# jackra1n/raytracer-rust

Measured on AMD Instinct MI355X. Metric: Msamples/s (pixels x spp / s) at 800x600x256spp; 1/2/4/8-GPU scaling, higher is better.
Workload: dtype f32; 1 GPU; cornell-box-800x600x256-d30; scene=data/scenes/tungsten/cornell-box/scene.json, width=800, height=600, spp=256, max_bounces=30, parallelism=row strips of 4 dealt round-robin over 1 GPU(s), frames_in_flight=1

## Files before the change

raytracer-rust_amd/csrc/device/rt_api.cpp:

```cpp
#include <hip/hip_runtime_api.h>

#include <algorithm>
#include <cmath>
#include <cstdio>
#include <cstdlib>
#include <cstring>
#include <map>
#include <mutex>
#include <new>
#include <stdexcept>
#include <string>
#include <thread>
#include <vector>

#include "../../../include/mi355rt.h"
#include "rt_device.h"
#include "rt_host.h"
#include "rt_query.h"

using namespace mi355rt;

namespace {

void row_tables(const std::vector<uint32_t>& rows, const std::vector<float>& cost, uint32_t groups, std::vector<uint32_t>& out) {
// ... 38 lines not shown
    uint32_t inline_steps = 0;
    uint32_t trav_min = 24;
    bool have_scene = false;
    mi355rt_settings settings{};
    DevCamera cam{};
    float miss[3] = {0.5f, 0.5f, 0.5f};
    uint32_t n_prims = 0, n_mats = 0; size_t n_nodes = 0;
    DevBuf<DevPrim> prims; DevBuf<DevMat> mats; DevBuf<DevNode> nodes; DevBuf<DevTri> tris;
    DevBuf<uint32_t> rows; DevBuf<float> radiance; DevBuf<uint32_t> counters; DevBuf<unsigned long long> stats;
    DevBuf<float> fold_stack;
    DevBuf<float> sky; uint32_t sky_w = 0, sky_h = 0;
    DevBuf<DevTexture> textures; DevBuf<uint32_t> texels;
    DevBuf<unsigned long long> wave_times; uint32_t wave_times_n = 0;
    std::vector<uint32_t> rows_host;
    std::vector<uint32_t> tables_host;
    bool rows_valid = false;
    std::vector<float> row_cost;
    int knob_row_order = -1;
    uint32_t order_groups = 0;
    hipEvent_t ev[3] = {nullptr, nullptr, nullptr};
    hipEvent_t done = nullptr; hipStream_t last_stream = nullptr; bool have_last = false;
    bool want_wave_times = false;
    DevBuf<unsigned long long> errword; unsigned long long* h_err = nullptr; unsigned long long err_reported = 0;
    uint32_t spin_limit_idle = SPIN_LIMIT_IDLE, spin_limit_entry = SPIN_LIMIT_ENTRY;
    uint32_t launched_variants = 0;
    int forced_variant = -1;
    int knob_inline_steps = -1;
    bool timing = false;
    std::vector<hipEvent_t> pool; size_t pool_used = 0;
    uint32_t timed_launches = 0;
// ... 24 lines not shown
    ctx->launched_variants = 0;
    for (const auto& w : waits) if ((now >> 32) & w.bit) which += std::string(which.empty() ? "" : "; ") + w.what;
    return fail(MI355RT_ERR_HIP, "kernel watchdog: " + std::to_string(n) + " wave(s) gave up a bounded wait " + (this_render ? "in this render" : "in an earlier render on this context") +
                                 " -- that image is incomplete [kernel(s) launched on this context since the last report: " + (kernels.empty() ? "?" : kernels) + "; wait: " + (which.empty() ? "?" : which) +
                                 "; limits: " + std::to_string(ctx->spin_limit_idle) + " idle polls, " + std::to_string(ctx->spin_limit_entry) + " polls of a ring entry]");
}

namespace {

uint32_t built_variants() {
    uint32_t mask = 0u;
    for (uint32_t v = 0; v < KERNEL_VARIANTS; ++v) if (render_ctr_variant_built(v)) mask |= 1u << v;
    return mask;
}

int build_device_scene(mi355rt_context* ctx, const mi355rt_scene* sc) {
    PreparedScene s;
    int rc = prepare_scene(sc, s); if (rc) return rc;
    const bool has_sky = sc->sky_rgb != nullptr;
    if ((rc = ctx->prims.ensure(s.prims.size()))) return rc;
    if ((rc = ctx->mats.ensure(sc->n_materials))) return rc;
    if ((rc = ctx->nodes.ensure(s.nodes.size()))) return rc;
    if ((rc = ctx->tris.ensure(s.tris.size()))) return rc;
    static_assert(sizeof(DevMat) == sizeof(mi355rt_material), "material layout is shared with the ABI");
    if (!s.prims.empty()) HIP_TRY(hipMemcpy(ctx->prims.p, s.prims.data(), s.prims.size() * sizeof(DevPrim), hipMemcpyHostToDevice));
    if (sc->n_materials) HIP_TRY(hipMemcpy(ctx->mats.p, sc->materials, sc->n_materials * sizeof(DevMat), hipMemcpyHostToDevice));
    if (!s.nodes.empty()) HIP_TRY(hipMemcpy(ctx->nodes.p, s.nodes.data(), s.nodes.size() * sizeof(DevNode), hipMemcpyHostToDevice));
    if (!s.tris.empty()) HIP_TRY(hipMemcpy(ctx->tris.p, s.tris.data(), s.tris.size() * sizeof(DevTri), hipMemcpyHostToDevice));
    ctx->n_prims = sc->n_primitives; ctx->n_mats = sc->n_materials; ctx->n_nodes = s.nodes.size();
    std::memcpy(ctx->miss, sc->miss_color, 12);
    ctx->sky_w = ctx->sky_h = 0;
// ... 8 lines not shown
        if ((rc = ctx->textures.ensure(sc->n_textures))) return rc;
        std::vector<DevTexture> table(sc->n_textures);
        size_t off = 0;
        for (uint32_t i = 0; i < sc->n_textures; ++i) {
            const mi355rt_texture& t = sc->textures[i];
            const size_t n = (size_t)t.width * t.height;
            HIP_TRY(hipMemcpy(ctx->texels.p + off, t.rgba8, n * 4, hipMemcpyHostToDevice));
            table[i] = DevTexture{ctx->texels.p + off, t.width, t.height};
            off += n;
        }
        HIP_TRY(hipMemcpy(ctx->textures.p, table.data(), table.size() * sizeof(DevTexture), hipMemcpyHostToDevice));
    }
    ctx->has_mesh = s.n_mesh_prims != 0;
    ctx->variant = choose_variant(s, ctx->forced_variant, built_variants());
    ctx->inline_steps = choose_inline_steps(s, ctx->knob_inline_steps);
    return MI355RT_OK;
}

std::mutex g_knob_mutex;
std::map<std::string, int> g_default_knobs;
int apply_knob(mi355rt_context* ctx, const std::string& name, int v) {
    if (name == "kernel") { if (v < -1 || v >= (int)KERNEL_VARIANTS) return fail(MI355RT_ERR_INVALID, "knob kernel"); ctx->forced_variant = v; }
    else if (name == "inline_steps") { if (v < -1 || v > 8) return fail(MI355RT_ERR_INVALID, "knob inline_steps"); ctx->knob_inline_steps = v; }
    else if (name == "grid_div") { if (v < 1 || v > 16) return fail(MI355RT_ERR_INVALID, "knob grid_div"); ctx->grid_div = (uint32_t)v; }
    else if (name == "guided_mult") { if (v < 1 || v > 64) return fail(MI355RT_ERR_INVALID, "knob guided_mult"); ctx->guided_mult = (uint32_t)v; }
    else if (name == "trav_min") { if (v < 1 || v > 64) return fail(MI355RT_ERR_INVALID, "knob trav_min"); ctx->trav_min = (uint32_t)v; }
    else if (name == "spin_idle") { if (v < 1) return fail(MI355RT_ERR_INVALID, "knob spin_idle"); ctx->spin_limit_idle = (uint32_t)v; }
    else if (name == "spin_entry") { if (v < 1) return fail(MI355RT_ERR_INVALID, "knob spin_entry"); ctx->spin_limit_entry = (uint32_t)v; }
    else if (name == "wave_times") ctx->want_wave_times = v != 0;
    else if (name == "row_order") { if (v < -1 || v > 1) return fail(MI355RT_ERR_INVALID, "knob row_order"); ctx->knob_row_order = v; }
    else return fail(MI355RT_ERR_INVALID, "unknown knob " + name);
    return MI355RT_OK;
}

}

extern "C" {

int mi355rt_debug_set_knob(mi355rt_context* ctx, const char* name, int value) {
    return guard([&]() -> int {
    if (ctx) return name ? apply_knob(ctx, name, value) : fail(MI355RT_ERR_INVALID, "knob name is null");
    std::lock_guard<std::mutex> g(g_knob_mutex);
    if (!name) { g_default_knobs.clear(); return MI355RT_OK; }
    mi355rt_context probe;
// ... 62 lines not shown
    delete ctx;
}

static int render_samples(mi355rt_context* ctx, const mi355rt_options* opt, uint32_t s0, uint32_t s1, void* d_accum,
                          void* d_out_packed, void* d_out_linear, void* hip_stream, mi355rt_stats* stats, unsigned long long* d_row_counters = nullptr);

int mi355rt_context_set_scene(mi355rt_context* ctx, const mi355rt_scene* scene, const mi355rt_camera* camera,
                              const mi355rt_settings* settings) {
    return guard([&]() -> int {
    if (!ctx) return fail(MI355RT_ERR_INVALID, "ctx is null");
    if (!camera) return fail(MI355RT_ERR_INVALID, "camera is null");
    int rc = check_settings(settings); if (rc) return rc;
    HIP_TRY(hipSetDevice(ctx->device));
    ctx->have_scene = false; ctx->rows_valid = false;
    ctx->query_rows_release();
    rc = build_device_scene(ctx, scene); if (rc) return rc;
    static_assert(sizeof(DevCamera) == sizeof(mi355rt_camera), "camera layout is shared with the ABI");
    std::memcpy(&ctx->cam, camera, sizeof(DevCamera));
    ctx->settings = *settings;
    ctx->have_scene = true;
    struct TimingOff { mi355rt_context* c; bool was; ~TimingOff() { c->timing = was; } } timing_off{ctx, ctx->timing};
    ctx->timing = false;
    struct ProbeScope {
        mi355rt_context* c; mi355rt_settings full; uint32_t variant; uint32_t* d_tmp = nullptr; unsigned long long* d_cnt = nullptr; bool committed = false;
        ProbeScope(mi355rt_context* ctx) : c(ctx), full(ctx->settings), variant(ctx->variant) {}
        ~ProbeScope() {
            c->settings = full; c->rows_valid = false;
            if (d_tmp) (void)hipFree(d_tmp);
            if (d_cnt) (void)hipFree(d_cnt);
            if (!committed) { c->variant = variant; c->have_scene = false; c->row_cost.clear(); }
        }
// ... 52 lines not shown
    if (ctx->have_last && ctx->last_stream != stream) HIP_TRY(hipStreamWaitEvent(stream, ctx->done, 0));
    const uint32_t rng_mode = opt ? opt->rng_mode : (uint32_t)MI355RT_RNG_CTR;
    uint32_t groups = WORK_SHARDS;
    {   const uint64_t spp_now = std::max<uint64_t>(1, (uint64_t)s1 - s0), pixels = (uint64_t)sel.rows.size() * st.width;
        const uint64_t ws = (opt && opt->workspace_bytes) ? opt->workspace_bytes : (32ull << 30);
        const uint64_t cap = std::max<uint64_t>(1, std::min<uint64_t>(ws / 12, (1ull << 31) - 16 * RUN_LIMIT) / spp_now);
        const uint64_t band_pixels = std::max<uint64_t>(1, std::min(cap, pixels));
        groups *= (uint32_t)std::min<uint64_t>(64, std::max<uint64_t>(1, (pixels + band_pixels - 1) / band_pixels)); }
    if (ctx->row_cost.empty() || rng_mode != MI355RT_RNG_CTR) groups = 0;
    const bool same_rows = ctx->rows_valid && sel.rows == ctx->rows_host && groups == ctx->order_groups;
    if (!same_rows) {
        if (ctx->have_last) HIP_TRY(hipEventSynchronize(ctx->done));
        ctx->rows_host.swap(sel.rows);
        static const std::vector<float> no_cost;
        row_tables(ctx->rows_host, groups ? ctx->row_cost : no_cost, groups, ctx->tables_host);
        ctx->order_groups = groups;
        ctx->rows_valid = false;
    }
    const bool fixed_aabb = opt && (opt->flags & MI355RT_FLAG_FIXED_AABB) != 0u;
    if (opt && (opt->flags & ~MI355RT_FLAG_FIXED_AABB) != 0u) return fail(MI355RT_ERR_INVALID, "options.flags has unknown bits");
    if (fixed_aabb && rng_mode != MI355RT_RNG_CTR) return fail(MI355RT_ERR_INVALID, "MI355RT_FLAG_FIXED_AABB needs MI355RT_RNG_CTR (the replay mode reproduces the reference as it is)");
    uint32_t variant = ctx->variant;
    if (fixed_aabb && ctx->has_mesh) variant = VARIANT_TABLE[variant].fixed_aabb;
    if ((ctx->n_prims == 0 || st.max_depth == 0) && VARIANT_TABLE[variant].family == FAMILY_LOCKSTEP && !(VARIANT_TABLE[variant].prims & (1u << MI355RT_PRIM_MESH)))
        variant = KERNEL_LOCKSTEP_MESH;
    const uint64_t seed = opt ? opt->seed : 0;
    const uint32_t n_rows = (uint32_t)ctx->rows_host.size();
    if (stats) { std::memset(stats, 0, sizeof *stats); stats->rows_rendered = n_rows; stats->kernel_vgprs = (uint32_t)ctx->vgprs[variant]; stats->kernel_sgprs = (uint32_t)ctx->sgprs; }
    if (n_rows == 0) return MI355RT_OK;

    if (!same_rows) {
        if ((rc = ctx->rows.ensure(3 * (size_t)n_rows))) return rc;
        HIP_TRY(hipMemcpyAsync(ctx->rows.p, ctx->tables_host.data(), 3 * (size_t)n_rows * sizeof(uint32_t), hipMemcpyHostToDevice, stream));
        ctx->rows_valid = true;
    }
    const uint32_t* d_rows_natural = ctx->rows.p;
    const uint32_t* d_rows_processing = ctx->rows.p + n_rows;
    const uint32_t* d_out_row = ctx->order_groups ? ctx->rows.p + 2 * (size_t)n_rows : nullptr;
    if ((rc = ctx->stats.ensure(STATS_WORDS))) return rc;
    HIP_TRY(hipMemsetAsync(ctx->stats.p, 0, STATS_WORDS * sizeof(unsigned long long), stream));

    double render_ms = 0, resolve_ms = 0, total_ms = 0;
    uint32_t n_bands = 0, grid_blocks = 0, block_threads = 0;

    if (rng_mode == MI355RT_RNG_REF) {
        if (d_accum || s0 != 0 || s1 != st.samples_per_pixel)
            return fail(MI355RT_ERR_INVALID, "progressive rendering needs MI355RT_RNG_CTR (the reference stream of a row is sequential over its pixels)");
        if ((rc = ctx->fold_stack.ensure((size_t)n_rows * std::max(st.max_depth, 1u) * 3))) return rc;
// ... 36 lines not shown

        RenderParams p{};
        p.prims = ctx->prims.p; p.mats = ctx->mats.p; p.nodes = ctx->nodes.p; p.tris = ctx->tris.p; p.rows = d_rows_processing;
        p.sky = ctx->sky_w ? ctx->sky.p : nullptr; p.sky_w = ctx->sky_w; p.sky_h = ctx->sky_h; p.textures = ctx->textures.p;
        p.radiance = ctx->radiance.p; p.stats = ctx->stats.p;
        p.n_prims = ctx->n_prims; p.n_mats = ctx->n_mats;
        std::memcpy(p.miss, ctx->miss, 12); p.cam = ctx->cam;
        p.width = st.width; p.height = st.height; p.spp = (uint32_t)spp; p.max_depth = st.max_depth;
        p.width_f = (float)st.width; p.height_f = (float)st.height;
        { volatile float one = 1.0f; p.inv_width_rn = one / p.width_f; p.inv_height_rn = one / p.height_f; }
        p.seed_lo = (uint32_t)seed; p.seed_hi = (uint32_t)(seed >> 32); p.sample0 = s0;
        magic_div((uint32_t)spp, p.spp_mul, p.spp_shift); magic_div(st.width, p.width_mul, p.width_shift);
        p.trav_min = ctx->trav_min; p.inline_steps = ctx->inline_steps;
        p.lds_nodes = (uint32_t)std::min<size_t>(ctx->n_nodes, LDS_NODE_CAP);
        p.err = ctx->errword.p; p.spin_limit_idle = ctx->spin_limit_idle; p.spin_limit_entry = ctx->spin_limit_entry;
        ResolveParams r{};
        r.radiance = ctx->radiance.p; r.out_packed = (uint32_t*)d_out_packed; r.out_linear = (float*)d_out_linear;
        r.spp = (uint32_t)spp; r.inv_spp = 1.0f / (float)s1;
        r.accum = (float*)d_accum; r.accum_load = s0 != 0 ? 1u : 0u;
        r.out_row = d_out_row; r.width = st.width; r.width_mul = p.width_mul; r.width_shift = p.width_shift;
        const uint32_t resident = std::max(1u, (uint32_t)(ctx->cu_count * ctx->blocks_per_cu[variant]) / ctx->grid_div);
        block_threads = VARIANT_TABLE[variant].block_threads;
        std::vector<float> band_ms;
        for (uint32_t b = 0; b < n_bands; ++b) {
            const uint64_t p0 = (uint64_t)b * band_pixels_max;
            const uint64_t np = std::min<uint64_t>(band_pixels_max, total_pixels - p0);
            p.band_pixel0 = (uint32_t)p0; p.band_samples = (uint32_t)(np * spp);
            p.batch_counter = ctx->counters.p + (size_t)b * ctr_words;
            if (d_row_counters) p.stats = d_row_counters + STATS_WORDS * (size_t)b;
            const bool wf = VARIANT_TABLE[variant].family == FAMILY_WAVEFRONT;
// ... 178 lines not shown
    if (!out_variant || !out_inline_steps || !n_prims || !n_nodes || !n_tris) return fail(MI355RT_ERR_INVALID, "debug_prepare_scene: null");
    if (forced_variant < -1 || forced_variant >= (int)KERNEL_VARIANTS) return fail(MI355RT_ERR_INVALID, "knob kernel");
    PreparedScene s;
    const int rc = prepare_scene(scene, s); if (rc) return rc;
    if ((prims && *n_prims < s.prims.size()) || (nodes && *n_nodes < s.nodes.size()) || (tris && *n_tris < s.tris.size())) return fail(MI355RT_ERR_INVALID, "debug_prepare_scene: capacity");
    if (prims && !s.prims.empty()) std::memcpy(prims, s.prims.data(), s.prims.size() * sizeof(DevPrim));
    if (nodes && !s.nodes.empty()) std::memcpy(nodes, s.nodes.data(), s.nodes.size() * sizeof(DevNode));
    if (tris && !s.tris.empty()) std::memcpy(tris, s.tris.data(), s.tris.size() * sizeof(DevTri));
    *n_prims = (uint32_t)s.prims.size(); *n_nodes = (uint32_t)s.nodes.size(); *n_tris = (uint32_t)s.tris.size();
    *out_variant = choose_variant(s, forced_variant, built_variants());
    *out_inline_steps = choose_inline_steps(s, -1);
    return MI355RT_OK;
    });
}

int mi355rt_debug_read_counters(mi355rt_context* ctx, unsigned long long* out40) {
    return guard([&]() -> int {
    if (!ctx || !out40 || !ctx->stats.p) return fail(MI355RT_ERR_INVALID, "no counters");
    HIP_TRY(hipSetDevice(ctx->device));
    HIP_TRY(hipMemcpy(out40, ctx->stats.p, STATS_WORDS * sizeof(unsigned long long), hipMemcpyDeviceToHost));
    return MI355RT_OK;
    });
}

int mi355rt_debug_read_row_tables(mi355rt_context* ctx, uint32_t* tables, uint32_t capacity_entries, uint32_t* n_rows, float* cost, uint32_t cost_capacity, uint32_t* n_cost) {
    return guard([&]() -> int {
    if (!ctx || !n_rows) return fail(MI355RT_ERR_INVALID, "null");
    const size_t n = ctx->rows_host.size();
    *n_rows = (uint32_t)n;
    if (tables) { if (capacity_entries < 3 * n || ctx->tables_host.size() != 3 * n) return fail(MI355RT_ERR_INVALID, "row tables: capacity"); std::memcpy(tables, ctx->tables_host.data(), 3 * n * sizeof(uint32_t)); }
// ... 248 lines not shown
```

raytracer-rust_amd/csrc/device/rt_device.h:

```cpp
#pragma once
#include <stdint.h>
#include "../../../include/mi355rt.h"

namespace mi355rt {

struct DevPrim {
    uint32_t kind, material, node_begin, run_end;
    float d[52];
    float mat0[4];
};
static_assert(sizeof(DevPrim) == 240, "DevPrim must stay 16-byte granular");
static_assert(offsetof(DevPrim, d) % 16 == 0, "DevPrim::d is read sixteen words at a time as a 16-byte aligned vector (rt_intersect.h load_rec16)");

struct DevMat {
    uint32_t kind; float albedo[3];
    float aux[3];  float p0;
    float p1;      float eta[3];
    float k[3];    uint32_t texture;
};
static_assert(sizeof(DevMat) == 64, "DevMat");

struct DevTexture { const uint32_t* rgba8; uint32_t width, height; };

struct DevNode { float bmin[3]; uint32_t a; float bmax[3]; uint32_t b; };
// ... 31 lines not shown
    DevCamera cam;
    uint32_t width, height, spp, max_depth;
    float width_f, height_f, inv_width_rn, inv_height_rn;
    uint32_t band_pixel0;
    uint32_t band_samples;
    uint32_t guided_div;
    uint32_t shard_samples;
    uint32_t seed_lo, seed_hi;
    uint32_t sample0;
    uint32_t spp_mul, spp_shift, width_mul, width_shift;
    uint32_t trav_min;
    uint32_t inline_steps;
    uint32_t lds_nodes;
    uint32_t spin_limit_idle;
    uint32_t spin_limit_entry;
};
enum : uint32_t { WAIT_WF_IDLE = 1u, WAIT_WF_RING = 2u, WAIT_WF_FOLLOWED = 4u };
constexpr uint32_t SPIN_LIMIT_IDLE = 1u << 22;
constexpr uint32_t SPIN_LIMIT_ENTRY = 1u << 20;

enum : uint32_t {
    KERNEL_LOCKSTEP = 0, KERNEL_LOCKSTEP_MESH = 1, KERNEL_STATE_MACHINE = 2, KERNEL_LOCKSTEP_SIMPLE = 3, KERNEL_STATE_MACHINE_FIXAABB = 4,
    KERNEL_RETIRED_5 = 5, KERNEL_RETIRED_6 = 6, KERNEL_WAVEFRONT = 7, KERNEL_WAVEFRONT_FIXAABB = 8, KERNEL_LOCKSTEP_NOSPEC = 9,
    KERNEL_WAVEFRONT_NOMETAL = 10, KERNEL_WAVEFRONT_MESHFREE = 11, KERNEL_WAVEFRONT_NOMETAL_IDENT = 12, KERNEL_WAVEFRONT_NOMETAL_SHALLOW = 13,
    KERNEL_LOCKSTEP_SIMPLE_QC = 14, KERNEL_VARIANTS = 15
};
constexpr uint32_t PRIMS_ALL = 0xFFFFFFFFu;
constexpr uint32_t PRIMS_MESH_FREE = PRIMS_ALL & ~(1u << MI355RT_PRIM_MESH);
constexpr uint32_t PRIMS_QUAD_CUBE = (1u << MI355RT_PRIM_QUAD) | (1u << MI355RT_PRIM_CUBE);
constexpr uint32_t WF_SHALLOW_NODES = 4096;
constexpr uint32_t MATBIT(uint32_t kind) { return 1u << kind; }
// ... 105 lines not shown
```

raytracer-rust_amd/csrc/device/rt_intersect.h:

```cpp
#pragma once
#include "rt_math.h"

namespace mi355rt {

struct Hit { float t; f3 p; f3 n; uint32_t mat_ff; float4 q0; };
constexpr uint32_t CAND_NONE = 0xFFFFFFFFu;
struct Cand {
    float t;
    uint32_t idx;
    float aux;
    uint32_t aux2;
};
DI void cand_reset(Cand& c) { c.t = __builtin_inff(); c.idx = CAND_NONE; c.aux = 0.f; c.aux2 = 0u; }
struct CandP : Cand { f3 po; };
DI void cand_reset(CandP& c) { cand_reset(static_cast<Cand&>(c)); c.po = mk(0.f, 0.f, 0.f); }

DI void set_face(Hit& h, f3 rd, f3 outward, uint32_t material) {
    bool front = dot(rd, outward) < 0.0f;
    h.n = front ? outward : -outward;
    h.mat_ff = material | (front ? 0x80000000u : 0u);
}

struct Probe { float t, aux; f3 po; };
typedef float rec16_t __attribute__((ext_vector_type(16), aligned(16)));
// ... 278 lines not shown
            set_face(h, rd, divf(h.p - mk(pr->d[0], pr->d[1], pr->d[2]), pr->d[3]), pr->material);
        } else if (kind == MI355RT_PRIM_PLANE) {
            h.p = ro + rd * c.t;
            set_face(h, rd, mk(pr->d[3], pr->d[4], pr->d[5]), pr->material);
        } else if (HAS_MESH) {
            f3 outward; finish_mesh(pr, reinterpret_cast<const float4*>(tris), c, ro, rd, h.p, outward);
            set_face(h, rd, outward, pr->material);
        }
    }
}

#undef MI_KIND
DI uint32_t prim_material_kind(const RenderParams& P, uint32_t idx) { return __float_as_uint(P.prims[idx].mat0[0]); }

template <bool HAS_MESH, uint32_t KINDS = PRIMS_ALL, class C>
DI void walk_list(cprim_t prims, uint32_t n_prims, const DevNode* __restrict__ nodes, const DevTri* __restrict__ tris, f3 ro, f3 rd, C& c) {
#define MI_KIND(k) (((KINDS >> (k)) & 1u) != 0u)
    uint32_t i = 0;
    while (i < n_prims) {
#define MI_RUN(KIND, CALL) if (i < n_prims && prims[i].kind == (KIND)) { const uint32_t end = min(prims[i].run_end, n_prims); do { CALL; } while (++i < end); }
        if (MI_KIND(MI355RT_PRIM_QUAD)) { MI_RUN(MI355RT_PRIM_QUAD,   hit_quad<!HAS_MESH>(prims + i, i, ro, rd, EPS, c)) }
        if (MI_KIND(MI355RT_PRIM_CUBE)) { MI_RUN(MI355RT_PRIM_CUBE,   hit_cube<!HAS_MESH>(prims + i, i, ro, rd, EPS, c)) }
        if (MI_KIND(MI355RT_PRIM_SPHERE)) { MI_RUN(MI355RT_PRIM_SPHERE, hit_sphere(prims + i, i, ro, rd, EPS, c)) }
        if (MI_KIND(MI355RT_PRIM_PLANE)) { MI_RUN(MI355RT_PRIM_PLANE,  hit_plane(prims + i, i, ro, rd, EPS, c)) }
        if (HAS_MESH) { MI_RUN(MI355RT_PRIM_MESH, hit_mesh(prims + i, i, nodes, tris, ro, rd, EPS, c)) }
        else if (KINDS == PRIMS_ALL) { if (i < n_prims && prims[i].kind >= MI355RT_PRIM_MESH) ++i; }
        else if (i < n_prims && ((KINDS >> prims[i].kind) & 1u) == 0u) ++i;
#undef MI_RUN
#undef MI_KIND
    }
}
template <bool HAS_MESH, bool CARRY_PO = false, uint32_t KINDS = PRIMS_ALL>
DI bool hit_scene(cprim_t prims, uint32_t n_prims, const DevNode* __restrict__ nodes, const DevTri* __restrict__ tris,
                  f3 ro, f3 rd, Hit& best) {
    typename std::conditional<CARRY_PO && !HAS_MESH, CandP, Cand>::type c; cand_reset(c);
    walk_list<HAS_MESH, KINDS>(prims, n_prims, nodes, tris, ro, rd, c);
    if (c.idx == CAND_NONE) return false;
    finish_hit<HAS_MESH, !HAS_MESH, !HAS_MESH, KINDS>((const DevPrim*)prims, tris, c, ro, rd, best);
    return true;
}


}
```

raytracer-rust_amd/csrc/device/rt_kernels.hip:

```cpp
#include <hip/hip_runtime.h>
#include <stdint.h>
#include <type_traits>
#include "rt_device.h"
#include "../../../include/mi355rt.h"

#include "rt_math.h"
#include "rt_rng.h"
#include "rt_intersect.h"
#include "rt_materials.h"

namespace mi355rt {

DI uint32_t mbcnt64(uint64_t mask) { return __builtin_amdgcn_mbcnt_hi((uint32_t)(mask >> 32), __builtin_amdgcn_mbcnt_lo((uint32_t)mask, 0u)); }
DI uint32_t wave_sum(uint32_t v) {
#pragma unroll
    for (int off = 32; off > 0; off >>= 1) v += __shfl_xor(v, off, 64);
    return v;
}
template <bool FENCED = true>
DI void wave_lds_handoff() {
    if constexpr (FENCED) __builtin_amdgcn_fence(__ATOMIC_RELEASE, "wavefront", "local");
    __builtin_amdgcn_wave_barrier();
    if constexpr (FENCED) __builtin_amdgcn_fence(__ATOMIC_ACQUIRE, "wavefront", "local");
}
// ... 376 lines not shown
    stock.dir = s_stock_dir + (threadIdx.x & ~63u); stock.key = s_stock_key + (threadIdx.x & ~63u);
    }
    PathState ps; ps.ro = mk(0, 0, 0); ps.rd = mk(0, 0, 1); ps.thr = mk(1, 1, 1); ps.sidx = 0; ps.ray_index = 0; ps.px = ps.py = 0;
    ps.rng.clear();
    bool live = false;
    uint32_t n_paths = 0, n_rays = 0;
    Prof prof; prof.begin();
#ifdef MI355RT_STAMPS
    const unsigned long long t_wave0 = __builtin_amdgcn_s_memrealtime();
    unsigned long long t_dry = 0ull; uint32_t drain_iters = 0, live_at_dry = 0;
#endif
    for (;;) {
        Hit h; bool hit = false;
        __builtin_amdgcn_s_setprio(1);
        uint32_t n_cam = 0u;
        if constexpr (PREHIT) {
            n_cam = wc.template refill_size<MI355RT_PREHIT_LOW>(P, lane);
            if (n_cam != 0u) {
                wave_lds_handoff();
                stock.park_a[lane] = make_float4(ps.ro.x, ps.ro.y, ps.ro.z, ps.rd.x); stock.park_b[lane] = make_float2(ps.rd.y, ps.rd.z);
                if (lane < n_cam) stock.camera(P, wc.next + lane, (wc.ring_head + wc.ring_count + lane) & 63u, ps.ro, ps.rd);
            }
        }
        if (n_cam != 0u ? lane < n_cam : live) hit = hit_scene<HAS_MESH, true, KINDS>(prims, P.n_prims, P.nodes, P.tris, ps.ro, ps.rd, h);
        prof.mark(1);
        if constexpr (PREHIT) {
            if (n_cam != 0u) {
                const bool cam = lane < n_cam;
                if (cam) { ++n_paths; ++n_rays; }
                wave_lds_handoff();
                wc.ring_count += stock.append(P, lane, wc.next, wc.ring_head + wc.ring_count, cam, hit, h, ps.rd);
                wave_lds_handoff();
                wc.next += n_cam;
                const float4 a = stock.park_a[lane]; const float2 b = stock.park_b[lane];
                ps.ro = mk(a.x, a.y, a.z); ps.rd = mk(a.w, b.x, b.y);
                prof.mark(2);
                continue;
            }
        }
// ... 246 lines not shown
```

raytracer-rust_amd/csrc/device/rt_prepare.cpp:

```cpp
#include "rt_prepare.h"

#include <algorithm>
#include <cmath>
#include <cstring>
#include <initializer_list>
#include <limits>
#include <utility>

using namespace mi355rt;

namespace {
thread_local std::string g_err;
}

namespace mi355rt {

int fail(int code, const std::string& msg) { g_err = msg; return code; }
int fail_noexcept(int code, const char* msg) noexcept { try { g_err.assign(msg); } catch (...) { g_err.clear(); } return code; }
std::string& last_error() { return g_err; }

int select_rows(const mi355rt_settings& st, const mi355rt_options* o, RowSel& sel) {
    uint32_t rb = 0, re = st.height, strip = 1, parts = 1, part = 0;
    if (o) {
        if (o->abi_version != MI355RT_ABI_VERSION && o->abi_version != 4u) return fail(MI355RT_ERR_INVALID, "options.abi_version mismatch");
// ... 260 lines not shown
                     : (rough && other_scatter && covers(KERNEL_WAVEFRONT_MESHFREE)) ? KERNEL_WAVEFRONT_MESHFREE
                     : covers(KERNEL_LOCKSTEP_NOSPEC) ? KERNEL_LOCKSTEP_NOSPEC : KERNEL_LOCKSTEP;
    }
    if (forced_variant >= 0) {
        const uint32_t v = (uint32_t)forced_variant;
        const bool ok = render_ctr_variant_built(v) && VARIANT_TABLE[v].forceable && covers(v) && kinds_covered(v) &&
                        !(VARIANT_TABLE[v].identity_meshes && !(has_mesh && all_meshes_identity));
        if (ok) chosen = v;
    }
    return chosen;
}

uint32_t choose_inline_steps(const PreparedScene& s, int knob) { return knob >= 0 ? (uint32_t)knob : (s.n_mesh_prims >= 2 ? 1u : 0u); }

}
```

raytracer-rust_amd/csrc/device/rt_prepare.h:

```cpp
#pragma once

#include <cstdint>
#include <new>
#include <stdexcept>
#include <string>
#include <vector>

#include "../../../include/mi355rt.h"
#include "rt_device.h"

namespace mi355rt {

int fail(int code, const std::string& msg);
int fail_noexcept(int code, const char* msg) noexcept;
std::string& last_error();

template <class F> int guard(F&& f) noexcept {
    try { return f(); }
    catch (const std::bad_alloc&) { return fail_noexcept(MI355RT_ERR_OOM, "host allocation failed (std::bad_alloc)"); }
    catch (const std::length_error&) { return fail_noexcept(MI355RT_ERR_OOM, "host allocation failed (std::length_error)"); }
    catch (const std::exception& e) {
        try { return fail(MI355RT_ERR_HIP, std::string("unexpected C++ exception: ") + e.what()); } catch (...) { return fail_noexcept(MI355RT_ERR_HIP, "unexpected C++ exception"); }
    }
    catch (...) { return fail_noexcept(MI355RT_ERR_HIP, "unexpected C++ exception"); }
// ... 7 lines not shown
struct PreparedScene {
    std::vector<DevNode> nodes; std::vector<DevTri> tris;
    std::vector<uint32_t> mesh_roots;
    std::vector<DevPrim> prims;
    uint64_t n_texels = 0;
    uint32_t scene_mats = 0u;
    uint32_t scene_prim_kinds = 0u;
    uint32_t n_mesh_prims = 0;
    bool all_meshes_identity = true, all_meshes_shallow = true;
};

int prepare_scene(const mi355rt_scene* sc, PreparedScene& out);
uint32_t choose_variant(const PreparedScene& s, int forced_variant, uint32_t built_mask);
uint32_t choose_inline_steps(const PreparedScene& s, int knob);

}
```

raytracer-rust_amd/device.py:

```python
import collections
import ctypes as C
import os

import numpy as np

from . import abi, build

EXPORTS = ["mi355rt_render", "mi355rt_render_multi", "mi355rt_render_progressive", "mi355rt_context_create", "mi355rt_context_destroy", "mi355rt_context_set_scene",
           "mi355rt_rows_selected", "mi355rt_context_render", "mi355rt_context_render_progressive", "mi355rt_context_set_timing", "mi355rt_context_read_timing",
           "mi355rt_context_check", "mi355rt_context_set_share", "mi355rt_last_error", "mi355rt_abi_version",
           "mi355rt_multi_context_create", "mi355rt_multi_context_destroy", "mi355rt_multi_context_set_scene", "mi355rt_multi_context_render",
           "mi355rt_multi_context_check", "mi355rt_multi_context_render_progressive", "mi355rt_render_progressive_multi",
           "mi355rt_context_trace_rays", "mi355rt_context_first_hits", "mi355rt_trace_rays"]

_lib = None
_extra = {}


def load(so):
    so = os.path.abspath(so)
    if so not in _extra:
        _extra[so] = _bind(so)
    return _extra[so]

# ... 126 lines not shown
        L.mi355rt_context_trace_rays.restype = C.c_int
        L.mi355rt_context_trace_rays.argtypes = [C.c_void_p, C.c_void_p, C.c_uint32, C.c_void_p, C.c_void_p]
        L.mi355rt_context_first_hits.restype = C.c_int
        L.mi355rt_context_first_hits.argtypes = [C.c_void_p, C.POINTER(abi.Options), C.c_void_p, C.c_void_p]
        L.mi355rt_trace_rays.restype = C.c_int
        L.mi355rt_trace_rays.argtypes = [C.POINTER(abi.Scene), C.c_void_p, C.c_uint32, C.c_void_p]
        L.mi355rt_debug_multi_part_ms.restype = C.c_int
        L.mi355rt_debug_multi_part_ms.argtypes = [C.c_void_p, C.POINTER(C.c_double), C.c_uint32, C.POINTER(C.c_uint32)]
        L.mi355rt_debug_set_knob.restype = C.c_int
        L.mi355rt_debug_set_knob.argtypes = [C.c_void_p, C.c_char_p, C.c_int]
        L.mi355rt_debug_has_variant.restype = C.c_int
        L.mi355rt_debug_has_variant.argtypes = [C.c_uint32]
        L.mi355rt_debug_prepare_scene.restype = C.c_int
        L.mi355rt_debug_prepare_scene.argtypes = [C.POINTER(abi.Scene), C.c_int, C.POINTER(C.c_uint32), C.POINTER(C.c_uint32),
                                                  C.c_void_p, C.POINTER(C.c_uint32), C.c_void_p, C.POINTER(C.c_uint32), C.c_void_p, C.POINTER(C.c_uint32)]
        if L.mi355rt_abi_version() != abi.ABI_VERSION:
            raise RuntimeError("libmi355rt.so ABI version does not match abi.py")
    return L


class RenderError(RuntimeError):
    def __init__(self, what, rc, library=None):
        super().__init__(f"{what} failed ({rc}): {(library or lib()).mi355rt_last_error().decode()}")
        self.rc = rc


def _check(rc, what, library=None):
    if rc != 0:
        raise RenderError(what, rc, library)

# ... 12 lines not shown
NODE_DTYPE = np.dtype([("bmin", "<f4", 3), ("a", "<u4"), ("bmax", "<f4", 3), ("b", "<u4")])
TRI_DTYPE = np.dtype([("v0", "<f4", 3), ("e1", "<f4", 3), ("e2", "<f4", 3), ("n", "<f4", 3)])
Prepared = collections.namedtuple("Prepared", "variant inline_steps prims nodes tris")


def prepare_scene(scene, forced_variant=-1, library=None):
    L = library or lib()
    sc = getattr(scene, "c", scene)
    variant, inline_steps, n_prims, n_nodes, n_tris = (C.c_uint32() for _ in range(5))
    _check(L.mi355rt_debug_prepare_scene(C.byref(sc), int(forced_variant), C.byref(variant), C.byref(inline_steps), None, C.byref(n_prims),
                                         None, C.byref(n_nodes), None, C.byref(n_tris)), "mi355rt_debug_prepare_scene", L)
    prims, nodes, tris = np.zeros(n_prims.value, PRIM_DTYPE), np.zeros(n_nodes.value, NODE_DTYPE), np.zeros(n_tris.value, TRI_DTYPE)
    _check(L.mi355rt_debug_prepare_scene(C.byref(sc), int(forced_variant), C.byref(variant), C.byref(inline_steps), prims.ctypes.data, C.byref(n_prims),
                                         nodes.ctypes.data, C.byref(n_nodes), tris.ctypes.data, C.byref(n_tris)), "mi355rt_debug_prepare_scene", L)
    return Prepared(variant.value, inline_steps.value, prims, nodes, tris)


def render(scene, camera, settings, options=None, want_linear=True, want_stats=True, library=None):
    L = library or lib()
    sc = getattr(scene, "c", scene)
    rows = len(abi.rows_selected(settings.height, options))
    W = settings.width
    packed = np.zeros((rows, W), np.uint32)
    linear = np.zeros((rows, W, 3), np.float32) if want_linear else None
    stats = abi.Stats() if want_stats else None
    _check(L.mi355rt_render(C.byref(sc), C.byref(camera), C.byref(settings),
                            C.byref(options) if options is not None else None,
                            packed.ctypes.data, linear.ctypes.data if want_linear else None,
                            C.byref(stats) if want_stats else None), "mi355rt_render", L)
    return packed, linear, stats
# ... 261 lines not shown
```

Measured before the change: 10270 Msamples/s.

## Cull primitives for camera rays using per-pixel projected coverage masks

Adds a host-side pass that projects each quad and cube primitive's corners into screen space and builds a per-pixel 32-bit mask of primitives that could be hit by primary rays. The masks are gathered per processed row, uploaded alongside the row tables, and used in the lockstep kernel to skip intersection tests for primitives not covering the pixel range of a camera-ray refill. This cuts per-ray intersection work on the first bounce for small scenes like the Cornell box. It adds a host pass and an upload of width-by-rows words, plus a scalar mask load per refill, and relies on conservative inflation and dilation to stay correct.

```diff
diff --git a/raytracer-rust_amd/csrc/device/rt_api.cpp b/raytracer-rust_amd/csrc/device/rt_api.cpp
--- a/raytracer-rust_amd/csrc/device/rt_api.cpp
+++ b/raytracer-rust_amd/csrc/device/rt_api.cpp
@@ -76,6 +76,8 @@
     DevBuf<unsigned long long> wave_times; uint32_t wave_times_n = 0;
     std::vector<uint32_t> rows_host;
     std::vector<uint32_t> tables_host;
+    std::vector<uint32_t> cam_mask_abs, cam_mask_host; uint32_t cam_mask_w = 0, cam_mask_h = 0;
+    int knob_cam_cull = -1;
     bool rows_valid = false;
     std::vector<float> row_cost;
     int knob_row_order = -1;
@@ -130,7 +132,7 @@
     return mask;
 }
 
-int build_device_scene(mi355rt_context* ctx, const mi355rt_scene* sc) {
+int build_device_scene(mi355rt_context* ctx, const mi355rt_scene* sc, const mi355rt_camera* camera, const mi355rt_settings* st) {
     PreparedScene s;
     int rc = prepare_scene(sc, s); if (rc) return rc;
     const bool has_sky = sc->sky_rgb != nullptr;
@@ -169,6 +171,13 @@
     ctx->has_mesh = s.n_mesh_prims != 0;
     ctx->variant = choose_variant(s, ctx->forced_variant, built_variants());
     ctx->inline_steps = choose_inline_steps(s, ctx->knob_inline_steps);
+    ctx->cam_mask_abs.clear(); ctx->cam_mask_host.clear();
+    if (ctx->variant == KERNEL_LOCKSTEP_SIMPLE_QC && ctx->knob_cam_cull != 0) {
+        static_assert(sizeof(DevCamera) == sizeof(mi355rt_camera), "camera layout is shared with the ABI");
+        DevCamera cam; std::memcpy(&cam, camera, sizeof cam);
+        build_camera_masks(s, cam, st->width, st->height, ctx->cam_mask_abs);
+        ctx->cam_mask_w = st->width; ctx->cam_mask_h = st->height;
+    }
     return MI355RT_OK;
 }
 
@@ -183,6 +192,7 @@
     else if (name == "spin_idle") { if (v < 1) return fail(MI355RT_ERR_INVALID, "knob spin_idle"); ctx->spin_limit_idle = (uint32_t)v; }
     else if (name == "spin_entry") { if (v < 1) return fail(MI355RT_ERR_INVALID, "knob spin_entry"); ctx->spin_limit_entry = (uint32_t)v; }
     else if (name == "wave_times") ctx->want_wave_times = v != 0;
+    else if (name == "cam_cull") { if (v < -1 || v > 1) return fail(MI355RT_ERR_INVALID, "knob cam_cull"); ctx->knob_cam_cull = v; }
     else if (name == "row_order") { if (v < -1 || v > 1) return fail(MI355RT_ERR_INVALID, "knob row_order"); ctx->knob_row_order = v; }
     else return fail(MI355RT_ERR_INVALID, "unknown knob " + name);
     return MI355RT_OK;
@@ -275,7 +285,7 @@
     HIP_TRY(hipSetDevice(ctx->device));
     ctx->have_scene = false; ctx->rows_valid = false;
     ctx->query_rows_release();
-    rc = build_device_scene(ctx, scene); if (rc) return rc;
+    rc = build_device_scene(ctx, scene, camera, settings); if (rc) return rc;
     static_assert(sizeof(DevCamera) == sizeof(mi355rt_camera), "camera layout is shared with the ABI");
     std::memcpy(&ctx->cam, camera, sizeof(DevCamera));
     ctx->settings = *settings;
@@ -358,6 +368,9 @@
         ctx->rows_host.swap(sel.rows);
         static const std::vector<float> no_cost;
         row_tables(ctx->rows_host, groups ? ctx->row_cost : no_cost, groups, ctx->tables_host);
+        ctx->cam_mask_host.clear();
+        if (!ctx->cam_mask_abs.empty() && ctx->cam_mask_w == st.width && ctx->cam_mask_h == st.height)
+            gather_camera_masks(ctx->cam_mask_abs, st.width, ctx->tables_host.data() + ctx->rows_host.size(), ctx->rows_host.size(), ctx->cam_mask_host);
         ctx->order_groups = groups;
         ctx->rows_valid = false;
     }
@@ -374,8 +387,10 @@
     if (n_rows == 0) return MI355RT_OK;
 
     if (!same_rows) {
-        if ((rc = ctx->rows.ensure(3 * (size_t)n_rows))) return rc;
+        if ((rc = ctx->rows.ensure(3 * (size_t)n_rows + ctx->cam_mask_host.size()))) return rc;
         HIP_TRY(hipMemcpyAsync(ctx->rows.p, ctx->tables_host.data(), 3 * (size_t)n_rows * sizeof(uint32_t), hipMemcpyHostToDevice, stream));
+        if (!ctx->cam_mask_host.empty())
+            HIP_TRY(hipMemcpyAsync(ctx->rows.p + 3 * (size_t)n_rows, ctx->cam_mask_host.data(), ctx->cam_mask_host.size() * sizeof(uint32_t), hipMemcpyHostToDevice, stream));
         ctx->rows_valid = true;
     }
     const uint32_t* d_rows_natural = ctx->rows.p;
@@ -442,6 +457,7 @@
         p.trav_min = ctx->trav_min; p.inline_steps = ctx->inline_steps;
         p.lds_nodes = (uint32_t)std::min<size_t>(ctx->n_nodes, LDS_NODE_CAP);
         p.err = ctx->errword.p; p.spin_limit_idle = ctx->spin_limit_idle; p.spin_limit_entry = ctx->spin_limit_entry;
+        p.cam_mask_off = (variant == KERNEL_LOCKSTEP_SIMPLE_QC && ctx->cam_mask_host.size() == (size_t)n_rows * st.width) ? 2u * n_rows : 0u;
         ResolveParams r{};
         r.radiance = ctx->radiance.p; r.out_packed = (uint32_t*)d_out_packed; r.out_linear = (float*)d_out_linear;
         r.spp = (uint32_t)spp; r.inv_spp = 1.0f / (float)s1;
@@ -650,6 +666,30 @@
     });
 }
 
+int mi355rt_debug_camera_masks(const mi355rt_scene* scene, const mi355rt_camera* camera, const mi355rt_settings* settings, const mi355rt_options* options,
+                               int forced_variant, uint32_t* out, uint64_t capacity, uint64_t* n) {
+    return guard([&]() -> int {
+    if (!camera || !n) return fail(MI355RT_ERR_INVALID, "debug_camera_masks: null");
+    if (forced_variant < -1 || forced_variant >= (int)KERNEL_VARIANTS) return fail(MI355RT_ERR_INVALID, "knob kernel");
+    int rc = check_settings(settings); if (rc) return rc;
+    PreparedScene s;
+    rc = prepare_scene(scene, s); if (rc) return rc;
+    std::vector<uint32_t> table, gathered;
+    if (choose_variant(s, forced_variant, built_variants()) == KERNEL_LOCKSTEP_SIMPLE_QC) {
+        DevCamera cam; std::memcpy(&cam, camera, sizeof cam);
+        build_camera_masks(s, cam, settings->width, settings->height, table);
+    }
+    if (options && !table.empty()) {
+        RowSel sel; rc = select_rows(*settings, options, sel); if (rc) return rc;
+        gather_camera_masks(table, settings->width, sel.rows.data(), sel.rows.size(), gathered);
+        table.swap(gathered);
+    }
+    *n = table.size();
+    if (out) { if (capacity < table.size()) return fail(MI355RT_ERR_INVALID, "debug_camera_masks: capacity"); if (!table.empty()) std::memcpy(out, table.data(), table.size() * sizeof(uint32_t)); }
+    return MI355RT_OK;
+    });
+}
+
 int mi355rt_debug_read_counters(mi355rt_context* ctx, unsigned long long* out40) {
     return guard([&]() -> int {
     if (!ctx || !out40 || !ctx->stats.p) return fail(MI355RT_ERR_INVALID, "no counters");
diff --git a/raytracer-rust_amd/csrc/device/rt_device.h b/raytracer-rust_amd/csrc/device/rt_device.h
--- a/raytracer-rust_amd/csrc/device/rt_device.h
+++ b/raytracer-rust_amd/csrc/device/rt_device.h
@@ -69,7 +69,9 @@
     uint32_t lds_nodes;
     uint32_t spin_limit_idle;
     uint32_t spin_limit_entry;
+    uint32_t cam_mask_off;
 };
+static_assert(sizeof(RenderParams) == 280, "RenderParams: the kernels' implicit arguments follow it (see cam_mask_off)");
 enum : uint32_t { WAIT_WF_IDLE = 1u, WAIT_WF_RING = 2u, WAIT_WF_FOLLOWED = 4u };
 constexpr uint32_t SPIN_LIMIT_IDLE = 1u << 22;
 constexpr uint32_t SPIN_LIMIT_ENTRY = 1u << 20;
diff --git a/raytracer-rust_amd/csrc/device/rt_intersect.h b/raytracer-rust_amd/csrc/device/rt_intersect.h
--- a/raytracer-rust_amd/csrc/device/rt_intersect.h
+++ b/raytracer-rust_amd/csrc/device/rt_intersect.h
@@ -316,11 +316,11 @@
 DI uint32_t prim_material_kind(const RenderParams& P, uint32_t idx) { return __float_as_uint(P.prims[idx].mat0[0]); }
 
 template <bool HAS_MESH, uint32_t KINDS = PRIMS_ALL, class C>
-DI void walk_list(cprim_t prims, uint32_t n_prims, const DevNode* __restrict__ nodes, const DevTri* __restrict__ tris, f3 ro, f3 rd, C& c) {
+DI void walk_list(cprim_t prims, uint32_t n_prims, const DevNode* __restrict__ nodes, const DevTri* __restrict__ tris, f3 ro, f3 rd, C& c, uint32_t pmask = ~0u) {
 #define MI_KIND(k) (((KINDS >> (k)) & 1u) != 0u)
     uint32_t i = 0;
     while (i < n_prims) {
-#define MI_RUN(KIND, CALL) if (i < n_prims && prims[i].kind == (KIND)) { const uint32_t end = min(prims[i].run_end, n_prims); do { CALL; } while (++i < end); }
+#define MI_RUN(KIND, CALL) if (i < n_prims && prims[i].kind == (KIND)) { const uint32_t end = min(prims[i].run_end, n_prims); do { if ((pmask >> i) & 1u) { CALL; } } while (++i < end); }
         if (MI_KIND(MI355RT_PRIM_QUAD)) { MI_RUN(MI355RT_PRIM_QUAD,   hit_quad<!HAS_MESH>(prims + i, i, ro, rd, EPS, c)) }
         if (MI_KIND(MI355RT_PRIM_CUBE)) { MI_RUN(MI355RT_PRIM_CUBE,   hit_cube<!HAS_MESH>(prims + i, i, ro, rd, EPS, c)) }
         if (MI_KIND(MI355RT_PRIM_SPHERE)) { MI_RUN(MI355RT_PRIM_SPHERE, hit_sphere(prims + i, i, ro, rd, EPS, c)) }
@@ -334,9 +334,9 @@
 }
 template <bool HAS_MESH, bool CARRY_PO = false, uint32_t KINDS = PRIMS_ALL>
 DI bool hit_scene(cprim_t prims, uint32_t n_prims, const DevNode* __restrict__ nodes, const DevTri* __restrict__ tris,
-                  f3 ro, f3 rd, Hit& best) {
+                  f3 ro, f3 rd, Hit& best, uint32_t pmask = ~0u) {
     typename std::conditional<CARRY_PO && !HAS_MESH, CandP, Cand>::type c; cand_reset(c);
-    walk_list<HAS_MESH, KINDS>(prims, n_prims, nodes, tris, ro, rd, c);
+    walk_list<HAS_MESH, KINDS>(prims, n_prims, nodes, tris, ro, rd, c, pmask);
     if (c.idx == CAND_NONE) return false;
     finish_hit<HAS_MESH, !HAS_MESH, !HAS_MESH, KINDS>((const DevPrim*)prims, tris, c, ro, rd, best);
     return true;
diff --git a/raytracer-rust_amd/csrc/device/rt_kernels.hip b/raytracer-rust_amd/csrc/device/rt_kernels.hip
--- a/raytracer-rust_amd/csrc/device/rt_kernels.hip
+++ b/raytracer-rust_amd/csrc/device/rt_kernels.hip
@@ -414,15 +414,21 @@
         Hit h; bool hit = false;
         __builtin_amdgcn_s_setprio(1);
         uint32_t n_cam = 0u;
+        uint32_t pmask = ~0u;
         if constexpr (PREHIT) {
             n_cam = wc.template refill_size<MI355RT_PREHIT_LOW>(P, lane);
             if (n_cam != 0u) {
+                if (P.cam_mask_off != 0u) {
+                    const uint32_t pix0 = fastdiv(wc.next, P.spp_mul, P.spp_shift), pix1 = fastdiv(wc.next + n_cam - 1u, P.spp_mul, P.spp_shift);
+                    const __attribute__((address_space(4))) uint32_t* cm = (const __attribute__((address_space(4))) uint32_t*)(P.rows) + P.cam_mask_off + P.band_pixel0;
+                    if (pix1 - pix0 <= 1u) pmask = cm[pix0] | cm[pix1];
+                }
                 wave_lds_handoff();
                 stock.park_a[lane] = make_float4(ps.ro.x, ps.ro.y, ps.ro.z, ps.rd.x); stock.park_b[lane] = make_float2(ps.rd.y, ps.rd.z);
                 if (lane < n_cam) stock.camera(P, wc.next + lane, (wc.ring_head + wc.ring_count + lane) & 63u, ps.ro, ps.rd);
             }
         }
-        if (n_cam != 0u ? lane < n_cam : live) hit = hit_scene<HAS_MESH, true, KINDS>(prims, P.n_prims, P.nodes, P.tris, ps.ro, ps.rd, h);
+        if (n_cam != 0u ? lane < n_cam : live) hit = hit_scene<HAS_MESH, true, KINDS>(prims, P.n_prims, P.nodes, P.tris, ps.ro, ps.rd, h, pmask);
         prof.mark(1);
         if constexpr (PREHIT) {
             if (n_cam != 0u) {
diff --git a/raytracer-rust_amd/csrc/device/rt_prepare.cpp b/raytracer-rust_amd/csrc/device/rt_prepare.cpp
--- a/raytracer-rust_amd/csrc/device/rt_prepare.cpp
+++ b/raytracer-rust_amd/csrc/device/rt_prepare.cpp
@@ -298,3 +298,114 @@
 uint32_t choose_inline_steps(const PreparedScene& s, int knob) { return knob >= 0 ? (uint32_t)knob : (s.n_mesh_prims >= 2 ? 1u : 0u); }
 
 }
+
+namespace {
+
+constexpr double MASK_INFLATE = 1e-3;
+constexpr double MASK_DILATE = 1.0;
+constexpr double MASK_TAN_MAX = 1e6;
+
+struct V3 { double x, y, z; };
+V3 v3(const float* p) { return V3{(double)p[0], (double)p[1], (double)p[2]}; }
+double dot(V3 a, V3 b) { return a.x * b.x + a.y * b.y + a.z * b.z; }
+V3 cross(V3 a, V3 b) { return V3{a.y * b.z - a.z * b.y, a.z * b.x - a.x * b.z, a.x * b.y - a.y * b.x}; }
+double maxabs(V3 a) { return std::max(std::fabs(a.x), std::max(std::fabs(a.y), std::fabs(a.z))); }
+
+bool solve_rows(V3 r0, V3 r1, V3 r2, V3 b, V3& x) {
+    const V3 c12 = cross(r1, r2), c20 = cross(r2, r0), c01 = cross(r0, r1);
+    const double det = dot(r0, c12), scale = maxabs(r0) * maxabs(r1) * maxabs(r2);
+    if (!std::isfinite(det) || !std::isfinite(scale) || !(std::fabs(det) > 1e-12 * scale)) return false;
+    x = V3{(b.x * c12.x + b.y * c20.x + b.z * c01.x) / det, (b.x * c12.y + b.y * c20.y + b.z * c01.y) / det, (b.x * c12.z + b.y * c20.z + b.z * c01.z) / det};
+    return std::isfinite(x.x) && std::isfinite(x.y) && std::isfinite(x.z);
+}
+
+int quad_corners(const mi355rt::DevPrim& p, V3* out) {
+    const V3 n = v3(p.d), base = v3(p.d + 4), e0 = v3(p.d + 7), e1 = v3(p.d + 10);
+    const double d = p.d[3], inv0 = p.d[13], inv1 = p.d[14];
+    const V3 r1 = V3{e0.x * inv0, e0.y * inv0, e0.z * inv0}, r2 = V3{e1.x * inv1, e1.y * inv1, e1.z * inv1};
+    int k = 0;
+    for (double a : {-MASK_INFLATE, 1.0 + MASK_INFLATE}) for (double b : {-MASK_INFLATE, 1.0 + MASK_INFLATE})
+        if (!solve_rows(n, r1, r2, V3{d, a + dot(base, r1), b + dot(base, r2)}, out[k++])) return 0;
+    return k;
+}
+int cube_corners(const mi355rt::DevPrim& p, V3* out) {
+    const float* m = p.d;
+    const V3 r0 = V3{m[0], m[3], m[6]}, r1 = V3{m[1], m[4], m[7]}, r2 = V3{m[2], m[5], m[8]}, c = v3(m + 9);
+    const double h = 0.5 + MASK_INFLATE;
+    int k = 0;
+    for (double x : {-h, h}) for (double y : {-h, h}) for (double z : {-h, h})
+        if (!solve_rows(r0, r1, r2, V3{x - c.x, y - c.y, z - c.z}, out[k++])) return 0;
+    return k;
+}
+
+}
+
+namespace mi355rt {
+
+void build_camera_masks(const PreparedScene& s, const DevCamera& cam, uint32_t width, uint32_t height, std::vector<uint32_t>& out) {
+    out.clear();
+    const size_t n_prims = s.prims.size();
+    if (n_prims == 0 || n_prims > 32 || width == 0 || height == 0) return;
+    out.assign((size_t)width * height, 0u);
+    const uint32_t all = n_prims == 32 ? 0xFFFFFFFFu : (1u << n_prims) - 1u;
+    uint32_t keep = 0u;
+    const V3 O = v3(cam.position), F = v3(cam.forward), R = v3(cam.right), U = v3(cam.true_up);
+    const double hw = cam.half_width, hh = cam.half_height, W = width, H = height;
+    const V3 row0 = V3{F.x, R.x, U.x}, row1 = V3{F.y, R.y, U.y}, row2 = V3{F.z, R.z, U.z};
+    const bool cam_ok = std::isfinite(hw) && std::isfinite(hh) && std::fabs(hw) > 0.0 && std::fabs(hh) > 0.0;
+    for (size_t i = 0; i < n_prims; ++i) {
+        const DevPrim& p = s.prims[i];
+        const uint32_t bit = 1u << i;
+        V3 corner[8];
+        const int n = !cam_ok ? 0 : p.kind == MI355RT_PRIM_QUAD ? quad_corners(p, corner) : p.kind == MI355RT_PRIM_CUBE ? cube_corners(p, corner) : 0;
+        if (n == 0) { keep |= bit; continue; }
+        double px[8], py[8];
+        int behind = 0; bool doubt = false;
+        for (int k = 0; k < n; ++k) {
+            V3 q;
+            if (!solve_rows(row0, row1, row2, V3{corner[k].x - O.x, corner[k].y - O.y, corner[k].z - O.z}, q)) { doubt = true; break; }
+            const double off = std::fabs(q.y) + std::fabs(q.z);
+            if (q.x < 0.0 && -q.x * MASK_TAN_MAX > off) { ++behind; continue; }
+            if (!(q.x > 0.0 && q.x * MASK_TAN_MAX > off)) { doubt = true; break; }
+            px[k] = (q.y / q.x / hw + 1.0) * 0.5 * W; py[k] = (1.0 - q.z / q.x / hh) * 0.5 * H;
+            if (!std::isfinite(px[k]) || !std::isfinite(py[k])) { doubt = true; break; }
+        }
+        if (!doubt && behind == n) continue;
+        if (doubt || behind != 0) { keep |= bit; continue; }
+        double ymin = py[0], ymax = py[0];
+        for (int k = 1; k < n; ++k) { ymin = std::min(ymin, py[k]); ymax = std::max(ymax, py[k]); }
+        const double ylo = std::floor(ymin - MASK_DILATE), yhi = std::floor(ymax + MASK_DILATE);
+        if (yhi < 0.0 || ylo > H - 1.0) continue;
+        const uint32_t y0 = (uint32_t)std::max(ylo, 0.0), y1 = (uint32_t)std::min(yhi, H - 1.0);
+        for (uint32_t y = y0; y <= y1; ++y) {
+            const double lo = (double)y - MASK_DILATE, hi = (double)y + 1.0 + MASK_DILATE;
+            double xmin = std::numeric_limits<double>::infinity(), xmax = -xmin;
+            for (int a = 0; a < n; ++a) for (int b = a; b < n; ++b) {
+                double xa = px[a], ya = py[a], xb = px[b], yb = py[b];
+                if (ya > yb) { std::swap(xa, xb); std::swap(ya, yb); }
+                if (yb < lo || ya > hi) continue;
+                const double dy = yb - ya;
+                double x_lo = xa, x_hi = xb;
+                if (dy > 0.0) {
+                    if (ya < lo) x_lo = xa + (xb - xa) * ((lo - ya) / dy);
+                    if (yb > hi) x_hi = xa + (xb - xa) * ((hi - ya) / dy);
+                }
+                xmin = std::min(xmin, std::min(x_lo, x_hi)); xmax = std::max(xmax, std::max(x_lo, x_hi));
+            }
+            if (!(xmin <= xmax)) continue;
+            const double fx0 = std::floor(xmin - MASK_DILATE), fx1 = std::floor(xmax + MASK_DILATE);
+            if (fx1 < 0.0 || fx0 > W - 1.0) continue;
+            const uint32_t x0 = (uint32_t)std::max(fx0, 0.0), x1 = (uint32_t)std::min(fx1, W - 1.0);
+            uint32_t* row = out.data() + (size_t)y * width;
+            for (uint32_t x = x0; x <= x1; ++x) row[x] |= bit;
+        }
+    }
+    if (keep != 0u) for (uint32_t& w : out) w |= keep & all;
+}
+
+void gather_camera_masks(const std::vector<uint32_t>& absolute, uint32_t width, const uint32_t* rows_processing, size_t n_rows, std::vector<uint32_t>& out) {
+    out.resize(n_rows * (size_t)width);
+    for (size_t j = 0; j < n_rows; ++j) std::memcpy(out.data() + j * width, absolute.data() + (size_t)rows_processing[j] * width, (size_t)width * sizeof(uint32_t));
+}
+
+}
diff --git a/raytracer-rust_amd/csrc/device/rt_prepare.h b/raytracer-rust_amd/csrc/device/rt_prepare.h
--- a/raytracer-rust_amd/csrc/device/rt_prepare.h
+++ b/raytracer-rust_amd/csrc/device/rt_prepare.h
@@ -45,4 +45,7 @@
 uint32_t choose_variant(const PreparedScene& s, int forced_variant, uint32_t built_mask);
 uint32_t choose_inline_steps(const PreparedScene& s, int knob);
 
+void build_camera_masks(const PreparedScene& s, const DevCamera& cam, uint32_t width, uint32_t height, std::vector<uint32_t>& out);
+void gather_camera_masks(const std::vector<uint32_t>& absolute, uint32_t width, const uint32_t* rows_processing, size_t n_rows, std::vector<uint32_t>& out);
+
 }
diff --git a/raytracer-rust_amd/device.py b/raytracer-rust_amd/device.py
--- a/raytracer-rust_amd/device.py
+++ b/raytracer-rust_amd/device.py
@@ -164,6 +164,9 @@
         L.mi355rt_debug_prepare_scene.restype = C.c_int
         L.mi355rt_debug_prepare_scene.argtypes = [C.POINTER(abi.Scene), C.c_int, C.POINTER(C.c_uint32), C.POINTER(C.c_uint32),
                                                   C.c_void_p, C.POINTER(C.c_uint32), C.c_void_p, C.POINTER(C.c_uint32), C.c_void_p, C.POINTER(C.c_uint32)]
+        L.mi355rt_debug_camera_masks.restype = C.c_int
+        L.mi355rt_debug_camera_masks.argtypes = [C.POINTER(abi.Scene), C.POINTER(abi.Camera), C.POINTER(abi.Settings), C.POINTER(abi.Options), C.c_int,
+                                                 C.c_void_p, C.c_uint64, C.POINTER(C.c_uint64)]
         if L.mi355rt_abi_version() != abi.ABI_VERSION:
             raise RuntimeError("libmi355rt.so ABI version does not match abi.py")
     return L
@@ -206,6 +209,21 @@
     _check(L.mi355rt_debug_prepare_scene(C.byref(sc), int(forced_variant), C.byref(variant), C.byref(inline_steps), prims.ctypes.data, C.byref(n_prims),
                                          nodes.ctypes.data, C.byref(n_nodes), tris.ctypes.data, C.byref(n_tris)), "mi355rt_debug_prepare_scene", L)
     return Prepared(variant.value, inline_steps.value, prims, nodes, tris)
+
+
+def camera_masks(scene, camera, settings, options=None, forced_variant=-1, library=None):
+    L = library or lib()
+    sc = getattr(scene, "c", scene)
+    n = C.c_uint64()
+    opt = C.byref(options) if options is not None else None
+    _check(L.mi355rt_debug_camera_masks(C.byref(sc), C.byref(camera), C.byref(settings), opt, int(forced_variant), None, 0, C.byref(n)),
+           "mi355rt_debug_camera_masks", L)
+    if n.value == 0:
+        return None
+    out = np.zeros(n.value, np.uint32)
+    _check(L.mi355rt_debug_camera_masks(C.byref(sc), C.byref(camera), C.byref(settings), opt, int(forced_variant), out.ctypes.data, out.size, C.byref(n)),
+           "mi355rt_debug_camera_masks", L)
+    return out.reshape(-1, settings.width)
 
 
 def render(scene, camera, settings, options=None, want_linear=True, want_stats=True, library=None):
```

Measured after the change: 10960 Msamples/s, median of 6. 1.07x the previous value.
